# COSIMA/cice4

Measured on AMD Instinct MI355X. Metric: EVP subcycles/sec, higher is better.
Workload: dtype f64; 1 GPU; gx1-size 320x384 rectangular synthetic grid, full ice cover, ncat=5, ndte=120; nx_global=320, ny_global=384, ndte=120, decomposition=1x1 j-slabs, one block per GPU, subcycles_in_the_most_common_launch=120, metrics_recomputed_from_HTN_HTE=True, active_T_cells=121980, active_U_cells=121280

## Files before the change

cice4_amd/csrc/capi.hip:

```cpp
#include <rccl/rccl.h>

#include <cmath>
#include <cstdlib>
#include <cstring>
#include <memory>
#include <algorithm>
#include <string>
#include <type_traits>
#include <vector>

#include "common.h"
#include "domain.h"
#include "evp.h"
#include "halo.h"
#include "atmo.h"
#include "therm.h"
#include "transport.h"

using namespace cice;

struct cice_ctx {
  int device = -1;
  hipStream_t stream = nullptr;
  std::string err;
// ... 98 lines not shown
    else CICE_HIP(hipGetDevice(&device));
    CICE_HIP(hipStreamCreateWithFlags(&stream, hipStreamNonBlocking));
    void* p = nullptr;
    CICE_HIP(hipMalloc(&p, 64));
    CICE_HIP(hipMemsetAsync(p, 0, 64, stream));
    CICE_HIP(hipStreamSynchronize(stream));
    CICE_HIP(hipFree(p));
  }
  void need_halo() {
    need_device();
    if (!halo) {
      CICE_REQUIRE(have_domain, "cice_domain_create has not been called");
      halo.reset(new Halo());
      frame_halo.reset();
      halo->init(dom, stream);
      if (comm) halo->set_comm((ncclComm*)comm, comm_rank, comm_nranks);
      if (link) halo->set_link(link, comm_rank, comm_nranks);
    }
  }
};

static std::string g_create_err;

#define CICE_TRY(ctx_) \
  cice_ctx* c_ = (ctx_); \
  if (!c_) return CICE_EINVAL; \
  try {                        \
    c_->bind_device();         \
    c_->fan.forked = false;
#define CICE_CATCH                                            \
  }                                                           \
  catch (const Error& e) {                                    \
    c_->err = e.msg;                                          \
    return e.code;                                            \
  }                                                           \
  catch (const std::exception& e) {                           \
    c_->err = e.what();                                       \
    return CICE_EINVAL;                                       \
  }                                                           \
  return CICE_OK;

__global__ __launch_bounds__(256) void k_diag_copy8(const double* __restrict__ src,
                                                    double* __restrict__ dst, size_t n) {
  size_t t = (size_t)blockIdx.x * blockDim.x + threadIdx.x;
  if (t < n) dst[t] = src[t] + 1.0;
}

__global__ __launch_bounds__(256) void k_diag_copy16(const double2* __restrict__ src,
                                                     double2* __restrict__ dst, size_t n2) {
  size_t t = (size_t)blockIdx.x * blockDim.x + threadIdx.x;
  if (t < n2) {
    double2 v = src[t];
// ... 588 lines not shown
  c_->evp->adopt_state(t.aicen.p, t.vicen.p, t.vsnon.p);
  CICE_CATCH
}
int cice_evp_pin_fields(cice_ctx* ctx, const cice_evp_fields* f) {
  CICE_TRY(ctx)
  NEED_EVP;
  CICE_REQUIRE(f, "NULL argument");
  const size_t n = (size_t)c_->dom.nblocks() * c_->dom.nx_block * c_->dom.ny_block;
  auto pin = [&](const void* h, size_t bytes) { c_->pin_range(h, bytes); };
  const double* r8[] = {f->aice, f->vice, f->vsno, f->aice0, f->strairxT, f->strairyT, f->uocn, f->vocn,
                        f->ss_tltx, f->ss_tlty, f->uvel, f->vvel, f->stressp_1, f->stressp_2, f->stressp_3,
                        f->stressp_4, f->stressm_1, f->stressm_2, f->stressm_3, f->stressm_4, f->stress12_1,
                        f->stress12_2, f->stress12_3, f->stress12_4, f->fm, f->strtltx, f->strtlty, f->strocnx,
                        f->strocny, f->strintx, f->strinty, f->strairx, f->strairy, f->strength, f->divu,
                        f->shear, f->rdg_conv, f->rdg_shear, f->prs_sig, f->strocnxT, f->strocnyT};
  for (const double* h : r8) pin(h, n * 8);
  pin(f->aicen, n * NCAT * 8);
  pin(f->vicen, n * NCAT * 8);
  pin(f->iceumask, n * 4);
  CICE_CATCH
}
int cice_evp_prepare(cice_ctx* ctx, double dt) { CICE_TRY(ctx) c_->chain_ready = false; NEED_EVP; c_->evp->forget_host_state(); c_->evp->prepare(dt); CICE_CATCH }
int cice_evp_subcycles(cice_ctx* ctx, int ksub0, int nsub, float* ms) {
  CICE_TRY(ctx) c_->chain_ready = false; NEED_EVP; c_->evp->forget_host_state(); c_->evp->subcycles(ksub0, nsub, ms); CICE_CATCH
}
int cice_evp_finish(cice_ctx* ctx) { CICE_TRY(ctx) c_->chain_ready = false; NEED_EVP; c_->evp->forget_host_state(); c_->evp->finish(); CICE_CATCH }
int cice_evp_download_stresses(cice_ctx* ctx, cice_evp_fields* f) {
  CICE_TRY(ctx) NEED_EVP; CICE_REQUIRE(f, "NULL argument"); c_->evp->download_stresses(*f); CICE_CATCH
}
int cice_evp_set_option(cice_ctx* ctx, const char* key, int value) {
  CICE_TRY(ctx) NEED_EVP; CICE_REQUIRE(key, "NULL key"); c_->evp->set_option(key, value); CICE_CATCH
}
int cice_evp_get_info(cice_ctx* ctx, const char* key, int* value) {
  CICE_TRY(ctx)
  NEED_EVP;
  CICE_REQUIRE(key && value, "NULL argument");
  if (!std::strcmp(key, "derive_metrics")) *value = c_->evp->derives_metrics() ? 1 : 0;
  else if (!std::strcmp(key, "waves")) *value = c_->evp->tile_waves();
  else if (!std::strcmp(key, "rows_per_wave")) *value = c_->evp->tile_rows();
  else if (!std::strcmp(key, "fused")) *value = c_->evp->can_fuse() ? 1 : 0;
  else if (!std::strcmp(key, "fused_waves")) *value = c_->evp->fused_waves();
  else if (!std::strcmp(key, "skew")) *value = c_->evp->can_skew() || c_->evp->can_skew_fold() ? 1 : 0;
  else if (!std::strcmp(key, "skew_fold")) *value = (!c_->evp->can_skew() && c_->evp->can_skew_fold()) || c_->evp->skew_joined_fold() ? 1 : 0;
  else if (!std::strcmp(key, "skew_joined")) *value = c_->evp->skew_joined() ? 1 : 0;
  else if (!std::strcmp(key, "skew_join_fold")) *value = c_->evp->join_fold_option() ? 1 : 0;
  else if (!std::strcmp(key, "skew_levels")) *value = c_->evp->skew_levels();
  else if (!std::strcmp(key, "skew_subs")) *value = c_->evp->skew_subs(c_->evp->skew_levels());
  else if (!std::strcmp(key, "skew_pairs")) *value = c_->evp->pairs_ok() ? 1 : 0;
  else if (!std::strcmp(key, "skew_fill")) *value = c_->evp->skew_rows_on() ? c_->evp->skew_fill_pct() : 0;
  else if (!std::strcmp(key, "resident_map")) *value = c_->evp->resident_map();
  else if (!std::strcmp(key, "skew_rowact")) *value = c_->evp->rowact_on() ? 1 : 0;
  else if (!std::strcmp(key, "skew_balance")) *value = c_->evp->skew_rows_on() && c_->evp->balance_on() ? 1 : 0;
  else if (!std::strcmp(key, "skew_balanced")) *value = (int)std::min<long long>(c_->evp->balanced_sweeps(), 2000000000LL);
  else if (!std::strcmp(key, "skew_trim_ext")) *value = (c_->evp->can_skew() && c_->evp->can_trim()) ? 1 : 0;
  else if (!std::strcmp(key, "skew_split")) *value = (c_->evp->can_skew() && c_->evp->can_split()) ? 1 : 0;
  else if (!std::strcmp(key, "skew_strips")) *value = c_->evp->skew_strips(c_->evp->skew_levels(), nullptr);
  else if (!std::strcmp(key, "skew_seg_rows")) *value = c_->evp->skew_seg_rows(c_->evp->skew_levels());
  else if (!std::strcmp(key, "resident")) *value = (c_->evp->can_reside() || c_->evp->can_reside_peer()) ? 1 : 0;
  else if (!std::strcmp(key, "resident_peer")) *value = c_->evp->can_reside_peer() ? 1 : 0;
// ... 875 lines not shown
int cice_transport_init(cice_ctx* ctx, const cice_transport_config* cfg, const cice_transport_grid* grid) {
  CICE_TRY(ctx)
  CICE_REQUIRE(cfg && grid, "NULL argument");
  c_->need_halo();
  c_->transport.reset(new Transport(c_->dom, *c_->halo, c_->stream, c_->fan));
  c_->transport->init(*cfg, *grid);
  CICE_CATCH
}

int cice_transport_remap(cice_ctx* ctx, double dt, const cice_transport_fields* f, int32_t* l_stop,
                         int32_t* istop, int32_t* jstop) {
  CICE_TRY(ctx)
  CICE_REQUIRE(c_->transport != nullptr, "cice_transport_init has not been called");
  CICE_REQUIRE(f, "NULL argument");
  if (c_->chain_on && c_->chain_ready && c_->evp && f->aice0 == c_->chain.aice0 && f->trcrn == c_->chain.trcrn &&
      f->vsnon == c_->chain.vsnon && f->eicen == c_->chain.eicen && f->esnon == c_->chain.esnon &&
      f->aicen == c_->chain_aicen && f->vicen == c_->chain_vicen && f->uvel == c_->chain_u && f->vvel == c_->chain_v)
    c_->transport->adopt(c_->evp->d_uv(), c_->evp->d_aicen(), c_->evp->d_vicen());
  c_->chain_ready = false;
  c_->transport->remap(dt, *f, l_stop, istop, jstop);
  CICE_CATCH
}

int cice_debug_skew_layout(int K, int S, int ncol, int cyclic, int* strips) {
  if (K < 2 || K > 8 || (S != 1 && S != 3) || ncol < 1) return -2;
  for (int shift = 0; shift < 2 * K + 4; ++shift)
    if (evp_skew_layout_ok(K, S, ncol, shift, cyclic != 0)) {
      const int ownw = 62 * S + 2 - 2 * K, f = ownw - 1 - shift, npos = ncol + 1;
      if (strips) *strips = npos <= f ? 1 : 1 + (npos - f + ownw - 1) / ownw;
      return shift;
    }
  return -1;
}

long long cice_debug_join_map(int nxg, int nyg, int bsx, int bsy, int ew, int ns, int32_t* map, long long cap) {
  try {
    return cice::join_map_debug(nxg, nyg, bsx, bsy, ew, ns, map, cap);
  } catch (...) {
    return -2;
  }
}

long long cice_debug_join_map_fold(int nxg, int nyg, int bsx, int bsy, int ew, int ns, int32_t* map, long long cap) {
  try {
    return cice::join_map_debug(nxg, nyg, bsx, bsy, ew, ns, map, cap, 1);
  } catch (...) {
// ... 60 lines not shown
```

cice4_amd/csrc/evp.h:

```cpp
#pragma once
#include <map>
#include <memory>
#include <functional>
#include <vector>

#include "common.h"
#include "domain.h"
#include "halo.h"
#include "join.h"

namespace cice {

struct SubArgs;
struct SkewArgs;

struct EvpScalars {
  double dtei, dte2T, denom1, denom2, rcon, ecci;
  int ndte, evp_damping;
  void set(double dt, int ndte_, int damping);
};

double balance_strip(int rows, int n, const int* e, const double* d, const double* w, const unsigned char* act, double* cost,
                     int* ne);

// ... 13 lines not shown
    subcycles(1, sc.ndte, nullptr);
    finish();
  }
  void run(double dt, cice_evp_fields& f, const std::function<void()>& while_looping = nullptr);
  void download_stresses(cice_evp_fields& f);
  void forget_host_state() { io_valid = false; }
  void set_option(const char* key, int value);
  void active_cells(long long* nt, long long* nu);
  long long debug_read(const char* what, long long* out, long long cap);
  bool derives_metrics() const;
  int tile_waves() const { return waves; }
  int tile_rows() const { return rows_per_wave; }
  bool can_reside() const;
  bool can_reside_peer() const;
  void peer_export(void* out[3]);
  void peer_connect(int side, void* xu0, void* xu1, void* rprog, long long peer_n);
  void peer_connect_rank(int rank, void* xu0, void* xu1, void* rprog, long long peer_n);
  std::vector<int> peer_ranks() const;
  int resident_waves() const;
  const double* d_uv() const { return uv[cur].p; }
  const double* d_aicen() const { return aicen.p; }
  const double* d_vicen() const { return vicen.p; }
  int last_launches = 0;
  bool peer_buffers_fine() const { return res_xu[0].fine && res_xu[1].fine && res_rprog.fine; }
  bool resident_dense() const;
  bool granules_in_use() const { return can_reside() && !halo.multi_rank() && granules_on() && !resident_dense(); }
  bool can_skew() const;
  bool can_join() const;
  bool skew_joined() const { return can_join() && can_skew(); }
  bool skew_joined_fold() const { return skew_joined() && img.g.fold; }
  bool join_fold_option() const { return join_fold_on; }
  bool can_split() const;
  bool skew_rows_on() const { return (skew_gen_pct > 0 || skew_fill_on() || balance_on()) && skew_seg_opt == 0; }
  bool skew_fill_on() const;
  int skew_fill_pct() const;
  bool rowact_on() const;
  int resident_map();
  bool balance_on() const;
  long long balanced_sweeps() const { return bal_sweeps; }
  bool can_trim() const;
  bool pairs_ok() const;
  bool can_skew_fold() const;
  int skew_levels() const;
  int skew_seg_rows(int K) const;
  int skew_strips(int K, int* shift) const;
  int skew_subs(int K) const;
// ... 66 lines not shown
  DevBuf<long long> skew_dbg;
  bool stamps_on = false;
  DevBuf<long long> stamp_buf;
  size_t stamp_used = 0;
  long long* stamp_buffer(size_t workgroups);
  int skew_stagger_ns = 0;
  int skew_k_opt = 0, skew_seg_opt = 0;
  long long skew_min_cells = 600000;
  int waves2 = 0;
  mutable int waves2_auto = 0;
  CopyFan& fan;
  bool resident_on = true, resident_failed = false;
  int res_w_opt = 0;
  bool res_dense = true;
  int res_prio = 2;
  int res_spin_us = 200000;
  int res_level = 0;
  hipEvent_t res_done_ev = nullptr;
  int res_retry_steps = 64;
  int res_retry_in = 0;
  int res_occ[5][2][6] = {};
  int res_gran = 1;
  unsigned* res_why = nullptr;
  bool res_sparse = false;
  bool granules_on() const;
  DevBuf<int32_t> res_src;
  DevBuf<double> res_xg;
  DevBuf<double> res_xgr;
  int resident_occupancy(int W, bool damp, bool peer);
  int res_w = 0, res_tiles = 0;
  unsigned res_epoch = 0;
  DevBuf<int32_t> res_deps;
  DevBuf<unsigned> res_prog;
  DevBuf<double> res_xu[2];
  bool skew_fold_on = true;
  void launch_subcycle_skew_fold(int ksub, int K);
  void ensure_band(int K);
  DevBuf<double> band[2];
  DevBuf<int32_t> blk_band;
  int band_k = 0;
  bool res_blocks_on = true;
  bool res_fold_on = true;
  void build_resident(int W);
  void build_resident_fold(std::vector<int32_t>& src_of, int tiles_x, int W);
  DevBuf<int32_t> res_ftab, res_deps2, res_fslot, res_ffwd;
  hipEvent_t res_t0 = nullptr, res_t1 = nullptr;
// ... 60 lines not shown

  void launch_subcycle(int ksub);
  void launch_subcycle_pair(int ksub);
  void launch_subcycle_skew(int ksub, int K, bool flip_and_halo = true, hipStream_t on = nullptr);
  void skew_args(SkewArgs& sa, int K);
  void skew_launch(const SkewArgs& sa, int K, bool last, int nt, hipStream_t s);
  bool split_on = false, in_capture = false;
  void build_split(int K);
  void launch_subcycle_skew_split(int ksub, int K);
  void launch_subcycle_skew_ext(int ksub, int K, int ext);
  bool trim_ext_on = true;
  int split_probe = 0;
  struct TileTab { int K, ext, S, nb, edge, total; bool split; DevBuf<int32_t> tab; };
  std::vector<std::unique_ptr<TileTab>> tile_tabs;
  const TileTab& tiles_for(int K, int ext, bool split);
  hipStream_t stream2 = nullptr;
  hipEvent_t ev_fork = nullptr, ev_join = nullptr;
  void launch_range(int ksub0, int nsub);
  void after_subcycle(int ksub);
  SubArgs make_args() const;
  void drop_graph();
};

bool evp_skew_layout_ok(int K, int S, int ncol, int shift, bool cyc);

#ifdef CICE4_AMD_AUSCOM
void evp_set_namelist(double cosw, double sinw, double dragio, int use_ocnslope);
#endif

}
```

cice4_amd/csrc/evp.hip:

```cpp
#include "evp.h"

#include <algorithm>
#include <array>
#include <cmath>
#include <cstdio>
#include <cstdlib>
#include <chrono>
#include <cstring>
#include <thread>

namespace cice {

using namespace K;

#ifdef CICE4_AMD_AUSCOM
__constant__ double cosw = 1.0, sinw = 0.0, dragw = dragio * rhow;
__constant__ int ocnslope = 0;

void evp_set_namelist(double cosw_, double sinw_, double dragio_, int use_ocnslope) {
  const double dragw_ = dragio_ * rhow;
  const int os = use_ocnslope != 0;
  CICE_HIP(hipMemcpyToSymbol(HIP_SYMBOL(cosw), &cosw_, 8));
  CICE_HIP(hipMemcpyToSymbol(HIP_SYMBOL(sinw), &sinw_, 8));
  CICE_HIP(hipMemcpyToSymbol(HIP_SYMBOL(dragw), &dragw_, 8));
// ... 2522 lines not shown
    if (i >= ilo && i <= ihi + 1 && j >= ojlo && j <= tjhi && a.icetmask[t] == 1) nt = 1;
    if (i >= ilo && i <= ihi && j >= ojlo && j <= ojhi && a.iceumask[t]) nu = 1;
  }
  for (int off = 32; off > 0; off >>= 1) {
    nt += __shfl_down(nt, off);
    nu += __shfl_down(nu, off);
  }
  __shared__ unsigned long long s_n[2][16];
  const int w = threadIdx.x >> 6;
  if ((threadIdx.x & 63) == 0) { s_n[0][w] = nt; s_n[1][w] = nu; }
  __syncthreads();
  if (threadIdx.x < 2) {
    unsigned long long sum = 0;
    for (int k = 0; k < (int)(blockDim.x >> 6); ++k) sum += s_n[threadIdx.x][k];
    if (sum) atomicAdd(&a.counters[threadIdx.x], sum);
  }
}

inline dim3 grid1(size_t n) { return dim3((unsigned)((n + 255) / 256)); }

}

Evp::~Evp() {
  drop_graph();
  if (res_done_ev) (void)hipEventDestroy(res_done_ev);
  for (hipEvent_t e : {res_t0, res_t1, sub_t0, sub_t1})
    if (e) (void)hipEventDestroy(e);
  if (ev_fork) (void)hipEventDestroy(ev_fork);
  if (ev_join) (void)hipEventDestroy(ev_join);
  if (stream2) (void)hipStreamDestroy(stream2);
  if (res_why) (void)hipHostFree(res_why);
}

void Evp::drop_graph() {
  if (graph_exec) (void)hipGraphExecDestroy(graph_exec);
  graph_exec = nullptr;
  graph_key[0] = -1;
}

void Evp::set_option(const char* key, int value) {
  if (!std::strcmp(key, "waves")) {
    CICE_REQUIRE(value == 4 || value == 8 || value == 16, "waves must be 4, 8 or 16");
    waves = value;
  } else if (!std::strcmp(key, "rows_per_wave")) {
    CICE_REQUIRE(value == 1 || value == 2 || value == 4 || value == 8, "rows_per_wave must be 1, 2, 4 or 8");
    rows_per_wave = value;
  } else if (!std::strcmp(key, "derive_metrics")) {
    derive_on = value != 0;
  } else if (!std::strcmp(key, "use_graph")) {
    use_graph = value != 0;
  } else if (!std::strcmp(key, "comm_graph")) {
    comm_graph = value != 0;
  } else if (!std::strcmp(key, "fuse")) {
    fuse_on = value != 0;
  } else if (!std::strcmp(key, "resident")) {
    resident_on = value != 0;
    if (value == 2) {
      resident_failed = false;
      res_level = 0;
      res_retry_in = 0;
    }
  } else if (!std::strcmp(key, "skew_fold")) {
    skew_fold_on = value != 0;
  } else if (!std::strcmp(key, "resident_blocks")) {
// ... 2231 lines not shown
  return nb;
}

int Evp::resident_occupancy(int W, bool damp, bool peer) {
  const int wi = W == 4 ? 0 : W == 6 ? 1 : W == 8 ? 2 : W == 11 ? 3 : 4;
  const bool fold = halo.has_fold();
  const bool gran = !peer && granules_on() && !resident_dense();
  int& c = res_occ[wi][damp][peer ? (fold ? 5 : 1) : (fold ? (gran ? 4 : 2) : (gran ? 3 : 0))];
  if (c == 0) {
    int nb = 0;
    switch (W) {
      case 4: nb = occ_res<4>(damp, peer, fold, gran); break;
      case 6: nb = occ_res<6>(damp, peer, fold, gran); break;
      case 8: nb = occ_res<8>(damp, peer, fold, gran); break;
      case 11: nb = occ_res<11>(damp, peer, fold, gran); break;
      case 12: nb = occ_res<12>(damp, peer, fold, gran); break;
      default: break;
    }
    c = nb > 0 ? nb : -1;
  }
  return c > 0 ? c : 0;
}

bool Evp::run_resident(int ksub0, int nsub) {
  const bool peer = halo.multi_rank();
  const int W = resident_waves();
  if (W != res_w || res_deps.n == 0 || peer != res_peer_built) {
    res_map_stale = true;
    try {
      if (peer) build_resident_peer(W);
      else build_resident(W);
    } catch (const Error& e) {
      if (peer) std::fprintf(stderr, "cice4_amd: resident EVP loop across ranks not possible: %s\n", e.msg.c_str());
      resident_failed = true;
      return false;
    }
  }
  if (res_epoch > 0x70000000u) {
    CICE_REQUIRE(!peer, "resident EVP loop across ranks: progress epoch exhausted (re-create the context)");
    res_prog.zero(stream);
    if (res_prog2.p) res_prog2.zero(stream);
    if (res_xg.p) res_xg.zero(stream);
    if (res_xgr.p) res_xgr.zero(stream);
    res_epoch = 0;
  }
  ResArgs r{};
// ... 30 lines not shown
      r.prp[sd] = peers[sd].rprog ? peers[sd].rprog + (size_t)peer_back[(size_t)sd] * RP_MAX * RES_STRIDE : nullptr;
    }
  }
  const bool dense = !peer && resident_dense();
  const bool gran = !peer && granules_on() && !dense && res_xg.p && res_src.p && (!halo.has_fold() || res_xgr.p);
  if (gran) {
    r.src = res_src.p;
    r.xg = res_xg.p;
    r.xg_half = (unsigned)(n * 32);
    r.xgr = res_xgr.p;
    static const int pd = [] { const char* e = std::getenv("CICE4_AMD_RESIDENT_POLL_DELAY"); return e ? std::atoi(e) : 2; }();
    static const int ps = [] { const char* e = std::getenv("CICE4_AMD_RESIDENT_POLL_SLEEP"); return e ? std::atoi(e) : 0; }();
    r.poll_delay = pd;
    r.poll_sleep = ps;
    static const int fk = [] { const char* e = std::getenv("CICE4_AMD_RESIDENT_FAKE_EW"); return e ? std::atoi(e) : 0; }();
    r.fake_ew = fk;
  } else {
    for (int k = 0; k < 2; ++k)
      CICE_HIP(hipMemcpyAsync(res_xu[k].p, uv[cur].p, 2 * n * 8, hipMemcpyDeviceToDevice, stream));
  }
  const dim3 g(8 * ((res_tiles + 7) / 8));
  const bool damp = sc.evp_damping != 0;
  {
    int ncu = 256, dev = 0;
    if (hipGetDevice(&dev) == hipSuccess) {
      int v = 0;
      if (hipDeviceGetAttribute(&v, hipDeviceAttributeMultiprocessorCount, dev) == hipSuccess && v > 0) ncu = v;
    }
    const int per_cu = resident_occupancy(W, damp, peer);
    if ((long long)per_cu * ncu < (long long)g.x) {
      std::fprintf(stderr, "cice4_amd: resident EVP loop not used: %u workgroups of %d wavefronts, the device holds %d x %d "
                           "of this kernel\n", g.x, W, per_cu, ncu);
      if (dense) res_level = 1;
      else resident_failed = true;
      return false;
    }
  }
  r.prio_mode = gran ? (res_prio == 2 ? 4 : res_prio) : (dense ? std::min(res_prio, 2) : 0);
  {
    static const bool top = [] { const char* e = std::getenv("CICE4_AMD_RESIDENT_PRIO_TOP"); return !(e && e[0] == '0'); }();
    r.prio_top = dense && top ? 1 : 0;
  }
  r.tile_map = nullptr;
  if (!peer && !halo.has_fold() && g.x <= 1024) {
    if (res_map.n == 0) { res_map.alloc(4); res_map_stale = true; }
    if (res_map_stale) {
      static const int force = [] { const char* e = std::getenv("CICE4_AMD_RESIDENT_MAP"); return e ? std::atoi(e) : -1; }();
      int ncu = 256, dev = 0;
      if (hipGetDevice(&dev) == hipSuccess) {
        int v = 0;
        if (hipDeviceGetAttribute(&v, hipDeviceAttributeMultiprocessorCount, dev) == hipSuccess && v > 0) ncu = v;
      }
      hipLaunchKernelGGL(k_res_choose_map, dim3(1), dim3(1024), 0, stream, r.a.tiles_x * r.a.tiles_y * r.a.nblocks, r.a.tiles_x,
                         r.a.tiles_y, W, dom.nx_block, dom.ny_block, std::max(1, ncu / 8), res_map_opt >= 0 ? res_map_opt : force,
                         (const int32_t*)blk.p, (const int32_t*)icetmask.p, (const int32_t*)iceumask.p, res_map.p, r.abort_flag + 7);
      res_map_stale = false;
    }
    r.tile_map = res_map.p;
  }
  {
    int ncu = 256, dev = 0;
    if (hipGetDevice(&dev) == hipSuccess) {
      int v = 0;
      if (hipDeviceGetAttribute(&v, hipDeviceAttributeMultiprocessorCount, dev) == hipSuccess && v > 0) ncu = v;
    }
    r.prio_div = std::max(1, ncu / 8);
  }
  r.stamps = stamp_buffer(3 * (size_t)g.x + 600);
  r.phases = r.stamps ? r.stamps + 4 * (size_t)g.x : nullptr;
  if (res_time_it) CICE_HIP(hipEventRecord(res_t0, stream));
  switch (W) {
    case 4: launch_res<4>(r, damp, peer, g, stream); break;
    case 6: launch_res<6>(r, damp, peer, g, stream); break;
    case 8: launch_res<8>(r, damp, peer, g, stream); break;
    case 11: launch_res<11>(r, damp, peer, g, stream); break;
    case 12: launch_res<12>(r, damp, peer, g, stream); break;
    default: throw Error{CICE_EINVAL, "resident_waves must be 4, 6, 8, 11 or 12"};
  }
  if (res_time_it) {
    CICE_HIP(hipEventRecord(res_t1, stream));
    res_timed = true;
  }
  if (const hipError_t le = hipGetLastError(); le != hipSuccess) {
    std::fprintf(stderr, "cice4_amd: resident EVP loop could not be launched (%s); this range runs as one launch per pair "
                         "of subcycles and so do later ones\n", hipGetErrorString(le));
    CICE_REQUIRE(!peer, "resident EVP loop across ranks: launch failed on this rank");
    resident_failed = true;
    return false;
  }
  unsigned aborted = 0;
  if (peer) {
    if (!res_done_ev) CICE_HIP(hipEventCreateWithFlags(&res_done_ev, hipEventDisableTiming));
    CICE_HIP(hipEventRecord(res_done_ev, stream));
    hipError_t q;
    while ((q = hipEventQuery(res_done_ev)) == hipErrorNotReady) std::this_thread::sleep_for(std::chrono::microseconds(20));
    CICE_HIP(q);
  }
  if (peer && res_peer_agree) halo.all_max_u32(r.abort_flag);
  if (!res_why) CICE_HIP(hipHostMalloc((void**)&res_why, 8 * sizeof(unsigned), hipHostMallocDefault));
  unsigned* why = res_why;
  CICE_HIP(hipMemcpyAsync(why, r.abort_flag, 8 * sizeof(unsigned), hipMemcpyDeviceToHost, stream));
  CICE_HIP(hipStreamSynchronize(stream));
  const int cover[3] = {0, (int)(why[7] >> 16), (int)(why[7] & 0xffffu)};
  if (r.tile_map && cover[2] > 0) {
    const int pct = (int)(100LL * cover[1] / cover[2]);
    if (pct < 50) res_sparse = true;
    else if (pct > 60) res_sparse = false;
  }
  aborted = why[0];
  res_epoch += (unsigned)nsub + (peer ? 3u : 0u);
  if (aborted && why[1]) {
    std::fprintf(stderr, "cice4_amd: rank %d: tile %u of %d gave up %s (subcycle %u of the launch, word wanted %u), producers "
                         "not heard from: lanes %08x%08x of its dependency list:", dom.rank, why[2], res_tiles,
                 why[1] == 1 ? "waiting for the neighbouring ranks' loops to begin" : why[1] == 4 ? "polling the granules of its halo" : "waiting for the producers of its halo",
                 why[3], why[6], why[5], why[4]);
    std::vector<int32_t> dl(RES_MAXDEP);
    CICE_HIP(hipMemcpy(dl.data(), res_deps.p + (size_t)why[2] * RES_MAXDEP, RES_MAXDEP * 4, hipMemcpyDeviceToHost));
    const unsigned long long ms = ((unsigned long long)why[5] << 32) | why[4];
    for (int l = 0; l < RES_MAXDEP; ++l)
      if ((ms >> l) & 1) {
        unsigned seen = 0;
        const int d = dl[l];
        const unsigned* wp = d <= -2 ? res_rprog.p + (size_t)(-2 - d) * RES_STRIDE : res_prog.p + (size_t)d * RES_STRIDE;
        CICE_HIP(hipMemcpy(&seen, wp, 4, hipMemcpyDeviceToHost));
        if (d <= -2) {
          const std::vector<int> pr = peer_ranks();
          const int sd = (-2 - d) / RP_MAX;
          std::fprintf(stderr, " [%d: rank %d's tile %d, word now %u]", l, sd < (int)pr.size() ? pr[(size_t)sd] : -1, (-2 - d) % RP_MAX, seen);
        } else {
          std::fprintf(stderr, " [%d: own tile %d, word now %u]", l, d, seen);
        }
      }
    std::fprintf(stderr, "\n");
  }
  if (aborted) {
    std::fprintf(stderr, "cice4_amd: resident EVP loop timed out (not every tile was resident%s); this range runs as one "
                         "launch per pair of subcycles%s\n", peer ? ", here or on another rank" : "",
                 dense ? ", later ones with one workgroup per CU" : " and so do later ones");
    if (dense) res_level = 1;
    else resident_failed = true;
    res_retry_in = (!peer || res_peer_agree) ? res_retry_steps : 0;
    res_prog.zero(stream);
    if (res_prog2.p) res_prog2.zero(stream);
    if (!peer && res_xg.p) res_xg.zero(stream);
    if (!peer && res_xgr.p) res_xgr.zero(stream);
    if (!peer) res_epoch = 0;
    return false;
  }
  cur = 1 - cur;
  ++flips;
  copies_identical = false;
  return true;
}

void Evp::launch_range(int ksub0, int nsub) {
  const bool fuse = can_fuse();
  const bool skew = can_skew(), skew_fold = !skew && can_skew_fold();
  const int K = skew_levels();
  const bool trim = skew && can_trim(), split = trim && can_split();
  const bool joined = skew && can_join();
  const bool pairs = skew && !joined && !trim && split_probe == 0 && pairs_ok();
  const int end = ksub0 + nsub - 1;
  for (int k = ksub0; k <= end;) {
    auto clear = [&](int len) {
      if (k + len - 1 > end) return false;
      if (dom.overlap > 0)
        for (int q = k; q < k + len - 1; ++q)
          if (q % dom.overlap == 0) return false;
      return true;
// ... 22 lines not shown
      }
      k += K;
    } else if (skew_fold && clear(K)) {
      launch_subcycle_skew_fold(k, K);
      k += K;
    } else if (fuse && clear(2)) {
      to_planes();
      launch_subcycle_pair(k);
      k += 2;
    } else {
      to_blocks();
      to_planes();
      launch_subcycle(k);
      k += 1;
    }
  }
  to_blocks();
  to_planes();
}

void Evp::subcycles(int ksub0, int nsub, float* elapsed_ms) {
  CICE_REQUIRE(prepared, "cice_evp_subcycles before cice_evp_prepare");
  CICE_REQUIRE(ksub0 >= 1 && nsub >= 0, "bad subcycle range");
  hipEvent_t &e0 = sub_t0, &e1 = sub_t1;
  const bool try_resident = nsub >= 2 && (can_reside() || can_reside_peer());
  if (elapsed_ms) {
    for (hipEvent_t* e : {&sub_t0, &sub_t1, &res_t0, &res_t1})
      if (!*e) CICE_HIP(hipEventCreate(e));
    if (!try_resident) CICE_HIP(hipEventRecord(e0, stream));
  }
  res_time_it = elapsed_ms != nullptr;
  res_timed = false;
  static const bool env_comm_graph = std::getenv("CICE4_AMD_COMM_GRAPH") != nullptr;
  bool graph_ok = use_graph && nsub > 1 && (!halo.multi_rank() || comm_graph || env_comm_graph);
  if (!can_skew() && can_skew_fold()) ensure_band(skew_levels());
  if (skew_joined_fold()) ensure_join_band(skew_levels());
  bool tuning = false;
  if ((can_skew() || can_skew_fold()) && skew_rows_on()) {
    const int K = skew_levels(), seg = skew_seg_rows(K);
    const int tiles_x = skew_strips(K, nullptr), tiles_y = ((sg().ny - 2) + seg - 1) / seg;
    build_skew_rows(K, tiles_x, tiles_y, sg().nb, seg);
    if (balance_on() && !(can_skew() && can_trim()) && nsub >= K && !(nsub >= 2 && (can_reside() || can_reside_peer()))) {
      if (bal_left == 0 && ++bal_since >= bal_every) {
        bal_left = BAL_AGAIN;
        bal_since = 0;
      }
      const size_t want = 2 * (size_t)(8 * ((std::max(tiles_x * tiles_y * sg().nb, bal_slots) + 7) / 8));
      if (bal_left > 0 && skew_dbg.n < want) skew_dbg.alloc(want);
      tuning = bal_left > 0;
    }
  }
  if (skew_joined())
    img_ensure();
  else if (pairs_ok())
    for (int k = 0; k < 2; ++k)
      if (st2[k].n < 14 * n) st2[k].alloc(14 * n);
  if ((can_skew() || can_skew_fold()) && (!skew_packed || packed_joined != can_join())) skew_pack();
  if (can_skew() && can_trim()) build_split(skew_levels());
  if (tuning) graph_ok = false;
  bool replayed = false;
  loop_launches = 0;
  if (try_resident) {
    replayed = run_resident(ksub0, nsub);
    if (replayed) loop_launches = 1;
    else res_timed = false;
    if (!replayed && elapsed_ms) CICE_HIP(hipEventRecord(e0, stream));
  }
  res_time_it = false;
  if (!replayed && graph_ok) {
    const int key[4] = {cur, ksub0, nsub,
                        ((((waves * 100 + rows_per_wave) * 2 + (derive_on ? 1 : 0)) * 64 + (fuse_on ? 32 : 0) + waves2) * 16 +
                         (can_skew() || can_skew_fold() ? skew_levels() : 0)) * 128 + (halo.generation() & 63) * 2 +
                            (copies_identical ? 1 : 0)};
    const int cur0 = cur;
    if (!graph_exec || std::memcmp(key, graph_key, sizeof(key)) != 0) {
      drop_graph();
      hipGraph_t gph = nullptr;
      bool capturing = false;
      try {
        CICE_HIP(hipStreamBeginCapture(stream, hipStreamCaptureModeThreadLocal));
        capturing = true;
        in_capture = true;
        flips = 0;
        loop_launches = 0;
        launch_range(ksub0, nsub);
        graph_flips = flips;
        graph_launches = loop_launches;
        capturing = false;
// ... 24 lines not shown
  last_launches = loop_launches;
  {
    static const bool stats = [] { const char* e = std::getenv("CICE4_AMD_STATS"); return e && e[0] == '1'; }();
    if (stats && stats_left > 0) {
      --stats_left;
      std::fprintf(stderr, "cice4_amd: subcycles %d..%d of evp(dt) on %d block(s): %d kernel launch(es)%s\n", ksub0, ksub0 + nsub - 1,
                   dom.nblocks(), last_launches, last_launches == 1 && nsub > 1 ? " (the whole loop in one launch, state in registers)" : "");
    }
  }
  if (elapsed_ms) {
    if (res_timed) {
      CICE_HIP(hipEventSynchronize(res_t1));
      CICE_HIP(hipEventElapsedTime(elapsed_ms, res_t0, res_t1));
    } else {
      CICE_HIP(hipEventRecord(e1, stream));
      CICE_HIP(hipEventSynchronize(e1));
      CICE_HIP(hipEventElapsedTime(elapsed_ms, e0, e1));
    }
  }
}

void Evp::finish() {
  CICE_REQUIRE(prepared, "cice_evp_finish before cice_evp_prepare");
  PrepArgs a{};
  a.nx = dom.nx_block; a.ny = dom.ny_block; a.nblocks = dom.nblocks(); a.n = n; a.blk = blk.p;
  a.iceumask = iceumask.p; a.uocn = uocn.p; a.vocn = vocn.p; a.u = uv[cur].p; a.v = uv[cur].p + n;
  a.aiu = aiu.p; a.strocnx = strocnx.p; a.strocny = strocny.p; a.strocnxT = strocnxT.p;
  a.strocnyT = strocnyT.p; a.tarea = tarea.p; a.uarea = uarea.p; a.fm = fm.p;
  const dim3 g = grid1(n), blk256(256);
  hipLaunchKernelGGL(k_finish, g, blk256, 0, stream, a);
  CICE_HIP(hipMemcpyAsync(work1.p, strocnxT.p, n * 8, hipMemcpyDeviceToDevice, stream));
  CICE_HIP(hipMemcpyAsync(work1.p + n, strocnyT.p, n * 8, hipMemcpyDeviceToDevice, stream));
  halo.update_r8(work1.p, 2, n, true, LOC_NECORNER, KIND_VECTOR);
  hipLaunchKernelGGL(k_to_tgrid2, g, blk256, 0, stream, a, (const double*)work1.p,
                     (const double*)(work1.p + n), strocnxT.p, strocnyT.p);
  CICE_HIP(hipGetLastError());
  CICE_HIP(hipStreamSynchronize(stream));
}

void Evp::stress_host(hipStream_t s, double dt, int ndte, int damping, int nx, int ny, int ksub,
                      int icellt, const int32_t* ti, const int32_t* tj, const double* uvel,
                      const double* vvel, const double* const grid10[10], const double* strength,
                      double* const sg[12], double* const diag[5], double* str) {
  const size_t np = (size_t)nx * ny;
  CICE_REQUIRE(icellt >= 0 && (size_t)icellt <= np, "icellt out of range");
  for (int e = 0; e < icellt; ++e)
// ... 83 lines not shown
```

include/cice4_amd.h:

```cpp
#ifndef CICE4_AMD_H
#define CICE4_AMD_H
#include <stddef.h>
#include <stdint.h>
#ifdef __cplusplus
extern "C" {
#endif

#define CICE_NCAT 5
#define CICE_NILYR 4
#define CICE_NSLYR 1
#define CICE_MAX_NTRCR 5

enum {
  CICE_OK = 0,
  CICE_EINVAL = -1,
  CICE_EDEVICE = -2,
  CICE_ECOMM = -3,
  CICE_EUNSUPPORTED = -4
};

typedef struct cice_ctx cice_ctx;

int cice_create(cice_ctx **ctx, int device);
int cice_device_count(void);
// ... 191 lines not shown

int cice_frzmlt_bottom_lateral(cice_ctx *ctx, int nx_block, int ny_block, int ilo, int ihi,
                               int jlo, int jhi, double dt, const double *aice,
                               const double *frzmlt, const double *eicen, const double *esnon,
                               const double *sst, const double *Tf, const double *strocnxT,
                               const double *strocnyT, double *Tbot, double *fbot,
                               double *rside);

typedef struct {
  int ntrcr;
  int trcr_depend[CICE_MAX_NTRCR];
} cice_transport_config;
typedef struct {
  const double *HTN, *HTE, *dxt, *dyt, *dxu, *dyu, *tarear, *hm;
} cice_transport_grid;
typedef struct {
  double *aice0, *aicen, *trcrn, *vicen, *vsnon, *eicen, *esnon;
  const double *uvel, *vvel;
} cice_transport_fields;
int cice_transport_init(cice_ctx *ctx, const cice_transport_config *cfg, const cice_transport_grid *grid);
int cice_transport_remap(cice_ctx *ctx, double dt, const cice_transport_fields *f, int32_t *l_stop,
                         int32_t *istop, int32_t *jstop);
int cice_debug_skew_layout(int K, int S, int ncol, int cyclic, int *strips);
long long cice_debug_join_map(int nxg, int nyg, int bsx, int bsy, int ew, int ns, int32_t *map, long long cap);
long long cice_debug_join_map_fold(int nxg, int nyg, int bsx, int bsy, int ew, int ns, int32_t *map, long long cap);
int cice_debug_balance_strip(int rows, int n, const int32_t *ends, const double *durations, const double *weights,
                             const unsigned char *rows_with_ice, int32_t *new_ends, double *total);
int cice_transport_chain(cice_ctx *ctx, const cice_transport_fields *fields);
int cice_transport_upwind_init(cice_ctx *ctx, const cice_transport_config *cfg, int nt_Tsfc, const double *HTE,
                               const double *HTN, const double *tarea);
int cice_transport_upwind(cice_ctx *ctx, double dt, const cice_transport_fields *f);
int cice_transport_debug(cice_ctx *ctx, int stop_stage, int which, double *out, long long *count);

const char *cice_build_flavour(void);
int cice_set_auscom(cice_ctx *ctx, double cosw, double sinw, double dragio, int use_ocnslope);
int cice_thermo_set_chio(cice_ctx *ctx, double chio);

#ifdef __cplusplus
}
#endif
#endif
```

Baseline: 205,500 subcycles/s.

## Defer resident EVP loop completion checks to avoid per-launch host synchronisation

Single-rank resident EVP subcycle launches no longer synchronise the stream to read the abort flag. Each launch queues an async copy of its status words into a pinned ring of records and returns straight away. Pending launches are retired (sync, check for timeouts, replay failed ranges non-resident) before finish, before any other API call, when the ring fills, or when the tables change. This removes a host round-trip per subcycles call so launches can run back-to-back, at the cost of more complex error recovery and replaying work after a late-detected abort. The device CU-count query is also cached.

```diff
diff --git a/cice4_amd/csrc/capi.hip b/cice4_amd/csrc/capi.hip
--- a/cice4_amd/csrc/capi.hip
+++ b/cice4_amd/csrc/capi.hip
@@ -144,12 +144,15 @@
 
 static std::string g_create_err;
 
-#define CICE_TRY(ctx_) \
+#define CICE_TRY_QUEUED(ctx_) \
   cice_ctx* c_ = (ctx_); \
   if (!c_) return CICE_EINVAL; \
   try {                        \
     c_->bind_device();         \
     c_->fan.forked = false;
+#define CICE_TRY(ctx_)  \
+  CICE_TRY_QUEUED(ctx_) \
+    if (c_->evp) c_->evp->retire_resident();
 #define CICE_CATCH                                            \
   }                                                           \
   catch (const Error& e) {                                    \
@@ -784,7 +787,7 @@
 }
 int cice_evp_prepare(cice_ctx* ctx, double dt) { CICE_TRY(ctx) c_->chain_ready = false; NEED_EVP; c_->evp->forget_host_state(); c_->evp->prepare(dt); CICE_CATCH }
 int cice_evp_subcycles(cice_ctx* ctx, int ksub0, int nsub, float* ms) {
-  CICE_TRY(ctx) c_->chain_ready = false; NEED_EVP; c_->evp->forget_host_state(); c_->evp->subcycles(ksub0, nsub, ms); CICE_CATCH
+  CICE_TRY_QUEUED(ctx) c_->chain_ready = false; NEED_EVP; c_->evp->forget_host_state(); c_->evp->subcycles(ksub0, nsub, ms); CICE_CATCH
 }
 int cice_evp_finish(cice_ctx* ctx) { CICE_TRY(ctx) c_->chain_ready = false; NEED_EVP; c_->evp->forget_host_state(); c_->evp->finish(); CICE_CATCH }
 int cice_evp_download_stresses(cice_ctx* ctx, cice_evp_fields* f) {
@@ -794,9 +797,14 @@
   CICE_TRY(ctx) NEED_EVP; CICE_REQUIRE(key, "NULL key"); c_->evp->set_option(key, value); CICE_CATCH
 }
 int cice_evp_get_info(cice_ctx* ctx, const char* key, int* value) {
-  CICE_TRY(ctx)
+  CICE_TRY_QUEUED(ctx)
   NEED_EVP;
   CICE_REQUIRE(key && value, "NULL argument");
+  if (!std::strcmp(key, "resident_pending")) {
+    *value = c_->evp->resident_pending();
+    return CICE_OK;
+  }
+  c_->evp->retire_resident();
   if (!std::strcmp(key, "derive_metrics")) *value = c_->evp->derives_metrics() ? 1 : 0;
   else if (!std::strcmp(key, "waves")) *value = c_->evp->tile_waves();
   else if (!std::strcmp(key, "rows_per_wave")) *value = c_->evp->tile_rows();
@@ -1718,6 +1726,15 @@
   CICE_CATCH
 }
 
+int cice_debug_resident_plan(int n, const uint32_t* word0, const int32_t* cur, const int32_t* flips, const int32_t* ident,
+                             int cur_now, int flips_now, int ident_now, int32_t out[5]) {
+  if (n < 0 || !out || (n > 0 && (!word0 || !cur || !flips || !ident))) return CICE_EINVAL;
+  int o[5];
+  evp_resident_plan(n, word0, cur, flips, ident, cur_now, flips_now, ident_now, o);
+  for (int k = 0; k < 5; ++k) out[k] = o[k];
+  return CICE_OK;
+}
+
 int cice_debug_skew_layout(int K, int S, int ncol, int cyclic, int* strips) {
   if (K < 2 || K > 8 || (S != 1 && S != 3) || ncol < 1) return -2;
   for (int shift = 0; shift < 2 * K + 4; ++shift)
diff --git a/cice4_amd/csrc/evp.h b/cice4_amd/csrc/evp.h
--- a/cice4_amd/csrc/evp.h
+++ b/cice4_amd/csrc/evp.h
@@ -59,6 +59,9 @@
   const double* d_aicen() const { return aicen.p; }
   const double* d_vicen() const { return vicen.p; }
   int last_launches = 0;
+  static constexpr int RES_RING = 16;
+  void retire_resident();
+  int resident_pending() const { return (int)res_pending.size(); }
   bool peer_buffers_fine() const { return res_xu[0].fine && res_xu[1].fine && res_rprog.fine; }
   bool resident_dense() const;
   bool granules_in_use() const { return can_reside() && !halo.multi_rank() && granules_on() && !resident_dense(); }
@@ -171,6 +174,16 @@
   int res_occ[5][2][6] = {};
   int res_gran = 1;
   unsigned* res_why = nullptr;
+  struct ResPending { int ksub0, nsub, cur, flips; bool copies_identical, dense, map; unsigned epoch0; int slot; };
+  std::vector<ResPending> res_pending;
+  bool res_async = true;
+  bool res_defer = false;
+  int res_ncu = 0;
+  int device_cus();
+  bool resident_tables_current() const;
+  void resident_cover(unsigned word7, bool map);
+  void resident_gave_up(const unsigned* why, bool dense, bool peer);
+  void run_range(int ksub0, int nsub, float* elapsed_ms, bool try_resident);
   bool res_sparse = false;
   bool granules_on() const;
   DevBuf<int32_t> res_src;
@@ -277,6 +290,9 @@
   void drop_graph();
 };
 
+void evp_resident_plan(int n, const unsigned* word0, const int* cur, const int* flips, const int* ident, int cur_now, int flips_now,
+                       int ident_now, int out[5]);
+
 bool evp_skew_layout_ok(int K, int S, int ncol, int shift, bool cyc);
 
 #ifdef CICE4_AMD_AUSCOM
diff --git a/cice4_amd/csrc/evp.hip b/cice4_amd/csrc/evp.hip
--- a/cice4_amd/csrc/evp.hip
+++ b/cice4_amd/csrc/evp.hip
@@ -2568,6 +2568,10 @@
 }
 
 Evp::~Evp() {
+  if (!res_pending.empty()) {
+    (void)hipStreamSynchronize(stream);
+    res_pending.clear();
+  }
   drop_graph();
   if (res_done_ev) (void)hipEventDestroy(res_done_ev);
   for (hipEvent_t e : {res_t0, res_t1, sub_t0, sub_t1})
@@ -2585,7 +2589,9 @@
 }
 
 void Evp::set_option(const char* key, int value) {
-  if (!std::strcmp(key, "waves")) {
+  if (!std::strcmp(key, "resident_async")) {
+    res_async = value != 0;
+  } else if (!std::strcmp(key, "waves")) {
     CICE_REQUIRE(value == 4 || value == 8 || value == 16, "waves must be 4, 8 or 16");
     waves = value;
   } else if (!std::strcmp(key, "rows_per_wave")) {
@@ -4863,6 +4869,102 @@
   return c > 0 ? c : 0;
 }
 
+int Evp::device_cus() {
+  if (res_ncu == 0) {
+    int dev = 0, v = 0;
+    res_ncu = 256;
+    if (hipGetDevice(&dev) == hipSuccess && hipDeviceGetAttribute(&v, hipDeviceAttributeMultiprocessorCount, dev) == hipSuccess && v > 0)
+      res_ncu = v;
+  }
+  return res_ncu;
+}
+
+bool Evp::resident_tables_current() const { return res_deps.n != 0 && !res_peer_built && resident_waves() == res_w; }
+
+void Evp::resident_cover(unsigned word7, bool map) {
+  const int cover[3] = {0, (int)(word7 >> 16), (int)(word7 & 0xffffu)};
+  if (map && cover[2] > 0) {
+    const int pct = (int)(100LL * cover[1] / cover[2]);
+    if (pct < 50) res_sparse = true;
+    else if (pct > 60) res_sparse = false;
+  }
+}
+
+void Evp::resident_gave_up(const unsigned* why, bool dense, bool peer) {
+  if (why[1]) {
+    std::fprintf(stderr, "cice4_amd: rank %d: tile %u of %d gave up %s (subcycle %u of the launch, word wanted %u), producers "
+                         "not heard from: lanes %08x%08x of its dependency list:", dom.rank, why[2], res_tiles,
+                 why[1] == 1 ? "waiting for the neighbouring ranks' loops to begin" : why[1] == 4 ? "polling the granules of its halo" : "waiting for the producers of its halo",
+                 why[3], why[6], why[5], why[4]);
+    std::vector<int32_t> dl(RES_MAXDEP);
+    CICE_HIP(hipMemcpy(dl.data(), res_deps.p + (size_t)why[2] * RES_MAXDEP, RES_MAXDEP * 4, hipMemcpyDeviceToHost));
+    const unsigned long long ms = ((unsigned long long)why[5] << 32) | why[4];
+    for (int l = 0; l < RES_MAXDEP; ++l)
+      if ((ms >> l) & 1) {
+        unsigned seen = 0;
+        const int d = dl[l];
+        const unsigned* wp = d <= -2 ? res_rprog.p + (size_t)(-2 - d) * RES_STRIDE : res_prog.p + (size_t)d * RES_STRIDE;
+        CICE_HIP(hipMemcpy(&seen, wp, 4, hipMemcpyDeviceToHost));
+        if (d <= -2) {
+          const std::vector<int> pr = peer_ranks();
+          const int sd = (-2 - d) / RP_MAX;
+          std::fprintf(stderr, " [%d: rank %d's tile %d, word now %u]", l, sd < (int)pr.size() ? pr[(size_t)sd] : -1, (-2 - d) % RP_MAX, seen);
+        } else {
+          std::fprintf(stderr, " [%d: own tile %d, word now %u]", l, d, seen);
+        }
+      }
+    std::fprintf(stderr, "\n");
+  }
+  std::fprintf(stderr, "cice4_amd: resident EVP loop timed out (not every tile was resident%s); this range runs as one "
+                       "launch per pair of subcycles%s\n", peer ? ", here or on another rank" : "",
+               dense ? ", later ones with one workgroup per CU" : " and so do later ones");
+  if (dense) res_level = 1;
+  else resident_failed = true;
+  res_retry_in = (!peer || res_peer_agree) ? res_retry_steps : 0;
+  res_prog.zero(stream);
+  if (res_prog2.p) res_prog2.zero(stream);
+  if (!peer && res_xg.p) res_xg.zero(stream);
+  if (!peer && res_xgr.p) res_xgr.zero(stream);
+  if (!peer) res_epoch = 0;
+}
+
+void evp_resident_plan(int n, const unsigned* word0, const int* cur, const int* flips, const int* ident, int cur_now, int flips_now,
+                       int ident_now, int out[5]) {
+  int k = 0;
+  while (k < n && word0[k] == 0u) ++k;
+  out[0] = k;
+  out[1] = n - k;
+  out[2] = k < n ? cur[k] : cur_now;
+  out[3] = k < n ? flips[k] : flips_now;
+  out[4] = k < n ? ident[k] : ident_now;
+}
+
+void Evp::retire_resident() {
+  if (res_pending.empty()) return;
+  CICE_HIP(hipStreamSynchronize(stream));
+  std::vector<ResPending> pend;
+  pend.swap(res_pending);
+  struct Sync { bool& d; bool was; ~Sync() { d = was; } } sync{res_defer, res_defer};
+  res_defer = false;
+  std::vector<unsigned> word0(pend.size());
+  std::vector<int> curs(pend.size()), flps(pend.size()), idents(pend.size());
+  for (size_t q = 0; q < pend.size(); ++q) {
+    word0[q] = res_why[8 * (size_t)pend[q].slot];
+    curs[q] = pend[q].cur; flps[q] = pend[q].flips; idents[q] = pend[q].copies_identical ? 1 : 0;
+  }
+  int plan[5];
+  evp_resident_plan((int)pend.size(), word0.data(), curs.data(), flps.data(), idents.data(), cur, flips, copies_identical ? 1 : 0, plan);
+  size_t k = 0;
+  for (; k < (size_t)plan[0]; ++k) resident_cover(res_why[8 * (size_t)pend[k].slot + 7], pend[k].map);
+  if (plan[1] == 0) return;
+  resident_gave_up(res_why + 8 * (size_t)pend[k].slot, pend[k].dense, false);
+  cur = plan[2];
+  flips = plan[3];
+  copies_identical = plan[4] != 0;
+  run_range(pend[k].ksub0, pend[k].nsub, nullptr, false);
+  for (++k; k < pend.size(); ++k) run_range(pend[k].ksub0, pend[k].nsub, nullptr, true);
+}
+
 bool Evp::run_resident(int ksub0, int nsub) {
   const bool peer = halo.multi_rank();
   const int W = resident_waves();
@@ -4939,11 +5041,7 @@
   const dim3 g(8 * ((res_tiles + 7) / 8));
   const bool damp = sc.evp_damping != 0;
   {
-    int ncu = 256, dev = 0;
-    if (hipGetDevice(&dev) == hipSuccess) {
-      int v = 0;
-      if (hipDeviceGetAttribute(&v, hipDeviceAttributeMultiprocessorCount, dev) == hipSuccess && v > 0) ncu = v;
-    }
+    const int ncu = device_cus();
     const int per_cu = resident_occupancy(W, damp, peer);
     if ((long long)per_cu * ncu < (long long)g.x) {
       std::fprintf(stderr, "cice4_amd: resident EVP loop not used: %u workgroups of %d wavefronts, the device holds %d x %d "
@@ -4963,11 +5061,7 @@
     if (res_map.n == 0) { res_map.alloc(4); res_map_stale = true; }
     if (res_map_stale) {
       static const int force = [] { const char* e = std::getenv("CICE4_AMD_RESIDENT_MAP"); return e ? std::atoi(e) : -1; }();
-      int ncu = 256, dev = 0;
-      if (hipGetDevice(&dev) == hipSuccess) {
-        int v = 0;
-        if (hipDeviceGetAttribute(&v, hipDeviceAttributeMultiprocessorCount, dev) == hipSuccess && v > 0) ncu = v;
-      }
+      const int ncu = device_cus();
       hipLaunchKernelGGL(k_res_choose_map, dim3(1), dim3(1024), 0, stream, r.a.tiles_x * r.a.tiles_y * r.a.nblocks, r.a.tiles_x,
                          r.a.tiles_y, W, dom.nx_block, dom.ny_block, std::max(1, ncu / 8), res_map_opt >= 0 ? res_map_opt : force,
                          (const int32_t*)blk.p, (const int32_t*)icetmask.p, (const int32_t*)iceumask.p, res_map.p, r.abort_flag + 7);
@@ -4976,11 +5070,7 @@
     r.tile_map = res_map.p;
   }
   {
-    int ncu = 256, dev = 0;
-    if (hipGetDevice(&dev) == hipSuccess) {
-      int v = 0;
-      if (hipDeviceGetAttribute(&v, hipDeviceAttributeMultiprocessorCount, dev) == hipSuccess && v > 0) ncu = v;
-    }
+    const int ncu = device_cus();
     r.prio_div = std::max(1, ncu / 8);
   }
   r.stamps = stamp_buffer(3 * (size_t)g.x + 600);
@@ -5005,7 +5095,18 @@
     resident_failed = true;
     return false;
   }
-  unsigned aborted = 0;
+  if (!res_why) CICE_HIP(hipHostMalloc((void**)&res_why, (RES_RING + 1) * 8 * sizeof(unsigned), hipHostMallocDefault));
+  if (res_defer && !peer) {
+    const int slot = (int)res_pending.size();
+    CICE_REQUIRE(slot < RES_RING, "resident EVP loop: more launches pending than records");
+    CICE_HIP(hipMemcpyAsync(res_why + 8 * (size_t)slot, r.abort_flag, 8 * sizeof(unsigned), hipMemcpyDeviceToHost, stream));
+    res_pending.push_back(ResPending{ksub0, nsub, cur, flips, copies_identical, dense, r.tile_map != nullptr, res_epoch, slot});
+    res_epoch += (unsigned)nsub;
+    cur = 1 - cur;
+    ++flips;
+    copies_identical = false;
+    return true;
+  }
   if (peer) {
     if (!res_done_ev) CICE_HIP(hipEventCreateWithFlags(&res_done_ev, hipEventDisableTiming));
     CICE_HIP(hipEventRecord(res_done_ev, stream));
@@ -5014,54 +5115,13 @@
     CICE_HIP(q);
   }
   if (peer && res_peer_agree) halo.all_max_u32(r.abort_flag);
-  if (!res_why) CICE_HIP(hipHostMalloc((void**)&res_why, 8 * sizeof(unsigned), hipHostMallocDefault));
-  unsigned* why = res_why;
+  unsigned* why = res_why + 8 * (size_t)RES_RING;
   CICE_HIP(hipMemcpyAsync(why, r.abort_flag, 8 * sizeof(unsigned), hipMemcpyDeviceToHost, stream));
   CICE_HIP(hipStreamSynchronize(stream));
-  const int cover[3] = {0, (int)(why[7] >> 16), (int)(why[7] & 0xffffu)};
-  if (r.tile_map && cover[2] > 0) {
-    const int pct = (int)(100LL * cover[1] / cover[2]);
-    if (pct < 50) res_sparse = true;
-    else if (pct > 60) res_sparse = false;
-  }
-  aborted = why[0];
+  resident_cover(why[7], r.tile_map != nullptr);
   res_epoch += (unsigned)nsub + (peer ? 3u : 0u);
-  if (aborted && why[1]) {
-    std::fprintf(stderr, "cice4_amd: rank %d: tile %u of %d gave up %s (subcycle %u of the launch, word wanted %u), producers "
-                         "not heard from: lanes %08x%08x of its dependency list:", dom.rank, why[2], res_tiles,
-                 why[1] == 1 ? "waiting for the neighbouring ranks' loops to begin" : why[1] == 4 ? "polling the granules of its halo" : "waiting for the producers of its halo",
-                 why[3], why[6], why[5], why[4]);
-    std::vector<int32_t> dl(RES_MAXDEP);
-    CICE_HIP(hipMemcpy(dl.data(), res_deps.p + (size_t)why[2] * RES_MAXDEP, RES_MAXDEP * 4, hipMemcpyDeviceToHost));
-    const unsigned long long ms = ((unsigned long long)why[5] << 32) | why[4];
-    for (int l = 0; l < RES_MAXDEP; ++l)
-      if ((ms >> l) & 1) {
-        unsigned seen = 0;
-        const int d = dl[l];
-        const unsigned* wp = d <= -2 ? res_rprog.p + (size_t)(-2 - d) * RES_STRIDE : res_prog.p + (size_t)d * RES_STRIDE;
-        CICE_HIP(hipMemcpy(&seen, wp, 4, hipMemcpyDeviceToHost));
-        if (d <= -2) {
-          const std::vector<int> pr = peer_ranks();
-          const int sd = (-2 - d) / RP_MAX;
-          std::fprintf(stderr, " [%d: rank %d's tile %d, word now %u]", l, sd < (int)pr.size() ? pr[(size_t)sd] : -1, (-2 - d) % RP_MAX, seen);
-        } else {
-          std::fprintf(stderr, " [%d: own tile %d, word now %u]", l, d, seen);
-        }
-      }
-    std::fprintf(stderr, "\n");
-  }
-  if (aborted) {
-    std::fprintf(stderr, "cice4_amd: resident EVP loop timed out (not every tile was resident%s); this range runs as one "
-                         "launch per pair of subcycles%s\n", peer ? ", here or on another rank" : "",
-                 dense ? ", later ones with one workgroup per CU" : " and so do later ones");
-    if (dense) res_level = 1;
-    else resident_failed = true;
-    res_retry_in = (!peer || res_peer_agree) ? res_retry_steps : 0;
-    res_prog.zero(stream);
-    if (res_prog2.p) res_prog2.zero(stream);
-    if (!peer && res_xg.p) res_xg.zero(stream);
-    if (!peer && res_xgr.p) res_xgr.zero(stream);
-    if (!peer) res_epoch = 0;
+  if (why[0]) {
+    resident_gave_up(why, dense, peer);
     return false;
   }
   cur = 1 - cur;
@@ -5130,8 +5190,26 @@
 void Evp::subcycles(int ksub0, int nsub, float* elapsed_ms) {
   CICE_REQUIRE(prepared, "cice_evp_subcycles before cice_evp_prepare");
   CICE_REQUIRE(ksub0 >= 1 && nsub >= 0, "bad subcycle range");
+  static const bool env_sync = [] { const char* e = std::getenv("CICE4_AMD_RESIDENT_ASYNC"); return e && e[0] == '0'; }();
+  auto queued = [&] { return res_async && !env_sync && !elapsed_ms && nsub >= 2 && !halo.multi_rank() && can_reside(); };
+  bool defer = queued();
+  if (!res_pending.empty() && (!defer || (int)res_pending.size() >= RES_RING || !resident_tables_current() || res_epoch > 0x70000000u)) {
+    retire_resident();
+    defer = queued();
+  }
+  res_defer = defer;
+  try {
+    run_range(ksub0, nsub, elapsed_ms, true);
+  } catch (...) {
+    res_defer = false;
+    throw;
+  }
+  res_defer = false;
+}
+
+void Evp::run_range(int ksub0, int nsub, float* elapsed_ms, bool try_resident_loop) {
   hipEvent_t &e0 = sub_t0, &e1 = sub_t1;
-  const bool try_resident = nsub >= 2 && (can_reside() || can_reside_peer());
+  const bool try_resident = try_resident_loop && nsub >= 2 && (can_reside() || can_reside_peer());
   if (elapsed_ms) {
     for (hipEvent_t* e : {&sub_t0, &sub_t1, &res_t0, &res_t1})
       if (!*e) CICE_HIP(hipEventCreate(e));
@@ -5172,6 +5250,10 @@
     replayed = run_resident(ksub0, nsub);
     if (replayed) loop_launches = 1;
     else res_timed = false;
+    if (!replayed && !res_pending.empty()) {
+      retire_resident();
+      loop_launches = 0;
+    }
     if (!replayed && elapsed_ms) CICE_HIP(hipEventRecord(e0, stream));
   }
   res_time_it = false;
@@ -5242,6 +5324,7 @@
 
 void Evp::finish() {
   CICE_REQUIRE(prepared, "cice_evp_finish before cice_evp_prepare");
+  retire_resident();
   PrepArgs a{};
   a.nx = dom.nx_block; a.ny = dom.ny_block; a.nblocks = dom.nblocks(); a.n = n; a.blk = blk.p;
   a.iceumask = iceumask.p; a.uocn = uocn.p; a.vocn = vocn.p; a.u = uv[cur].p; a.v = uv[cur].p + n;
diff --git a/include/cice4_amd.h b/include/cice4_amd.h
--- a/include/cice4_amd.h
+++ b/include/cice4_amd.h
@@ -237,6 +237,8 @@
 int cice_transport_remap(cice_ctx *ctx, double dt, const cice_transport_fields *f, int32_t *l_stop,
                          int32_t *istop, int32_t *jstop);
 int cice_debug_skew_layout(int K, int S, int ncol, int cyclic, int *strips);
+int cice_debug_resident_plan(int n, const uint32_t *word0, const int32_t *cur, const int32_t *flips, const int32_t *ident,
+                             int cur_now, int flips_now, int ident_now, int32_t out[5]);
 long long cice_debug_join_map(int nxg, int nyg, int bsx, int bsy, int ew, int ns, int32_t *map, long long cap);
 long long cice_debug_join_map_fold(int nxg, int nyg, int bsx, int bsy, int ew, int ns, int32_t *map, long long cap);
 int cice_debug_balance_strip(int rows, int n, const int32_t *ends, const double *durations, const double *weights,
```

Result: faster. 209,700 subcycles/s, median of 6 (+2.0%).
